# lijiaman/egoego_release

Measured on AMD Instinct MI355X. Metric: diffusion-steps/sec (B=256, T=120, 22-joint), higher is better.
Workload: dtype i8x3 + bf16x3 (attention layer, fc, FFN and linear_out: 2 x int8 slices per operand, int32 accumulate; embed: split-bf16, fp32 accumulate)

## Files before the change

egoego_release_amd/csrc/tail_fused.h:

```cpp
#pragma once
#include <type_traits>

#include "gemm.h"

#ifndef TAIL_ABLATE
#define TAIL_ABLATE 0
#endif
#ifndef TAIL_RING1
#define TAIL_RING1 4
#endif
#ifndef TAIL_RING_IO
#define TAIL_RING_IO 4
#endif
#ifndef TAIL8_RING
#define TAIL8_RING 4
#endif
#ifndef TAIL8_RING_FC
#define TAIL8_RING_FC 4
#endif

struct TailArgs {
    const __bf16* o;
    size_t o_plane;
    int HD16;
    const __bf16* wfc;
    size_t wfc_plane;
    EpiResLN<2, 4, 0> ln1;
    const __bf16* w1;
    size_t w1_plane;
    EpiTiled<true, 2> relu;
    const __bf16* w2;
    size_t w2_plane;
    EpiResLN<2, 4, 0> ln2;
    int fc8, H;
    const int8_t* o8;
    size_t o8_plane;
    const float* o_scale;
    const int8_t* wfc8;
    size_t wfc8_plane;
    const float* s_wfc;
    const int8_t* wfc8_3;
    int ffn8;
    const int8_t* w1_8;
    const int8_t* w2_8;
    size_t w8_plane;
    const float* s_w1;
    const float* s_w2;
    EpiReluQ8<4, 0> relu8;
    int stop;
    unsigned* outlier;
    int outlier_rows;
    EG_DBG(unsigned long long* trace;)
};

static constexpr int tail_smem_bytes(int TT, int NWV = 4) { return TT * 32 * 1024 + 3 * TT * NWV * 32 * TT * 4; }
static constexpr int TAIL_PAR_BYTES = 10 * 512 * 4;

using tail_rsrc = __amdgpu_buffer_rsrc_t;
EG_D tail_rsrc tail_make_rsrc(const void* p, size_t bytes) {
    return __builtin_amdgcn_make_buffer_rsrc((void*)p, 0, (int)(bytes < 0x7fffffffu ? bytes : 0x7fffffffu), 0x00020000);
}
EG_D i32x4 tail_load(tail_rsrc r, int voff, unsigned soff) {
    return __builtin_bit_cast(i32x4, __builtin_amdgcn_raw_buffer_load_b128(r, voff, soff, 0));
}

template <int FT, int TT, int RING, bool LAST, int DP, int NKS = 8, bool I8 = false, bool WLO0 = false>
struct TailChunk {
    using AccT = typename std::conditional<I8, I8Acc, f32x16>::type;
    static constexpr int PD = RING - 1, NW = FT * 2;
    static constexpr int NWL = WLO0 ? FT : NW;
    static_assert(!WLO0 || I8, "int8 slices only");
    static_assert(NKS == 8 || (LAST && DP == 0), "only the last chunk may be short");
    static_assert(RING == 2 || RING == 4 || RING == 8, "ring slots must divide the 8 k-steps of a chunk");
    static constexpr int n_ops(int s) { return ((s + PD < NKS || !LAST) ? NWL : 0) + (s == 0 ? DP : 0); }
    static constexpr int after_dma() {
        int n = 0;
        for (int s = 1; s < 8; ++s) n += n_ops(s);
        return n < 63 ? n : 63;
    }
    static constexpr int allowed(int ks) {
        int n = 0;
        if (ks < PD) {
            n += (PD - 1 - ks) * NWL;
            for (int s = 0; s < ks; ++s) n += n_ops(s);
        } else {
            n += ks - PD == 0 ? DP : 0;
            for (int s = ks - PD + 1; s < ks; ++s) n += n_ops(s);
        }
        return n < 63 ? n : 63;
    }
    template <int G>
    static EG_D void mma(i32x4 w, i32x4 a, f32x16& c) {
        if (TAIL_ABLATE & 8) return;
        c = __builtin_amdgcn_mfma_f32_32x32x16_bf16(__builtin_bit_cast(bf16x8, w), __builtin_bit_cast(bf16x8, a), c, 0, 0, 0);
    }
    template <int G>
    static EG_D void mma(i32x4 w, i32x4 a, I8Acc& c) {
        if (TAIL_ABLATE & 8) return;
        i32x16& d = G == 2 ? c.h : c.m;
        d = __builtin_amdgcn_mfma_i32_32x32x32_i8(w, a, d, 0, 0, 0);
    }

    template <int KS, class Dma>
    static EG_D void step(AccT (&acc)[FT][TT], i32x4 (&wq)[RING][NW], i32x4 (&ah)[2][TT], i32x4 (&al)[TT], tail_rsrc wr,
                          const unsigned (&wcur)[NW], const unsigned (&wnext)[NW], const char* act, int act_plane, int lane, Dma& dma) {
        constexpr int cur = KS & 1;
        asm volatile("" ::: "memory");
        wait_counts<allowed(KS), (KS == 0 ? 0 : TT)>();
        __builtin_amdgcn_sched_barrier(0);
        if (KS + PD < NKS || !LAST) {
            constexpr int kn = KS + PD;
#pragma unroll
            for (int q = 0; q < NW; ++q)
                if (!(TAIL_ABLATE & 1) && !(WLO0 && (q & 1))) wq[kn % RING][q] = tail_load(wr, lane * 16, kn < 8 ? wcur[q] + (kn << 10) : wnext[q] + ((kn & 7) << 10));
        }
        if (KS == 0 && DP) {
#pragma unroll
            for (int d = 0; d < DP; ++d)
                if (!(TAIL_ABLATE & 4)) dma(d);
        }
        if (KS < NKS - 1) {
#pragma unroll
            for (int j = 0; j < TT; ++j)
                if (!(TAIL_ABLATE & 2)) ah[cur ^ 1][j] = *(const i32x4*)(act + ((j * 8 + KS + 1) << 10) + lane * 16);
        }
        __builtin_amdgcn_sched_barrier(0);
        const i32x4(&w)[NW] = wq[KS % RING];
        if (!WLO0) {
#pragma unroll
            for (int i = 0; i < FT; ++i)
#pragma unroll
                for (int j = 0; j < TT; ++j) mma<0>(w[2 * i + 1], ah[cur][j], acc[i][j]);
        }
        asm volatile("" ::: "memory");
        wait_counts<63, (KS < NKS - 1 ? TT : 0)>();
        __builtin_amdgcn_sched_barrier(0);
#pragma unroll
        for (int i = 0; i < FT; ++i)
#pragma unroll
            for (int j = 0; j < TT; ++j) mma<1>(w[2 * i], al[j], acc[i][j]);
        __builtin_amdgcn_sched_barrier(0);
        if (KS < NKS - 1) {
#pragma unroll
            for (int j = 0; j < TT; ++j)
                if (!(TAIL_ABLATE & 2)) al[j] = *(const i32x4*)(act + act_plane + ((j * 8 + KS + 1) << 10) + lane * 16);
        }
        __builtin_amdgcn_sched_barrier(0);
#pragma unroll
        for (int i = 0; i < FT; ++i)
#pragma unroll
            for (int j = 0; j < TT; ++j) mma<2>(w[2 * i], ah[cur][j], acc[i][j]);
        __builtin_amdgcn_sched_barrier(0);
    }

    template <class Dma>
    static EG_D void run(AccT (&acc)[FT][TT], i32x4 (&wq)[RING][NW], tail_rsrc wr, const unsigned (&wcur)[NW],
                         const unsigned (&wnext)[NW], const char* act, int act_plane, int lane, Dma dma) {
        i32x4 ah[2][TT], al[TT];
#pragma unroll
        for (int j = 0; j < TT; ++j) {
            ah[0][j] = *(const i32x4*)(act + ((j * 8) << 10) + lane * 16);
            al[j] = *(const i32x4*)(act + act_plane + ((j * 8) << 10) + lane * 16);
        }
        step<0>(acc, wq, ah, al, wr, wcur, wnext, act, act_plane, lane, dma);
        if (NKS > 1) step<1>(acc, wq, ah, al, wr, wcur, wnext, act, act_plane, lane, dma);
        if (NKS > 2) step<2>(acc, wq, ah, al, wr, wcur, wnext, act, act_plane, lane, dma);
        if (NKS > 3) step<3>(acc, wq, ah, al, wr, wcur, wnext, act, act_plane, lane, dma);
        if (NKS > 4) step<4>(acc, wq, ah, al, wr, wcur, wnext, act, act_plane, lane, dma);
        if (NKS > 5) step<5>(acc, wq, ah, al, wr, wcur, wnext, act, act_plane, lane, dma);
        if (NKS > 6) step<6>(acc, wq, ah, al, wr, wcur, wnext, act, act_plane, lane, dma);
        if (NKS > 7) step<7>(acc, wq, ah, al, wr, wcur, wnext, act, act_plane, lane, dma);
        if (DP) {
            asm volatile("" ::: "memory");
            wait_counts<after_dma(), 15>();
        }
    }
};

template <int FT, int TT, int RING, bool REM2 = false, bool I8 = false, int NWAVES = 4, bool WLO0 = false>
struct DirectGemm {
    using AccT = typename std::conditional<I8, I8Acc, f32x16>::type;
    static constexpr int NW = 2 * FT, PD = RING - 1;
    static constexpr int CH_PLANE = TT * 8 * 1024, CH_BYTES = 2 * CH_PLANE;
    static constexpr int DMA_PIECES = 16 * TT / NWAVES;
    static constexpr int SMEM_BYTES = 2 * CH_BYTES;

    struct NoPost {
        EG_D void operator()(int) const {}
    };
    struct NoPre {
        EG_D void operator()() const {}
    };
    template <class Mark, class Post = NoPost, class Pre = NoPre>
    static EG_D void run(AccT (&acc)[FT][TT], const __bf16* in, size_t in_plane, int K16, const __bf16* w, size_t w_plane, char* act,
                         int tt0, int wave, int lane, Mark mark, int wtile0 = -1, Post post = Post{}, Pre pre = Pre{}) {
        const int wt0 = wtile0 >= 0 ? wtile0 : wave * FT;
        i32x4 wq[RING][NW];
        const tail_rsrc wr = tail_make_rsrc(w, w_plane * 4);
        const tail_rsrc ir = tail_make_rsrc((const char*)in + (((size_t)tt0 * (size_t)K16) << 10), 0x7fffffffu);
        const unsigned wpb = (unsigned)(w_plane * 2), ipb = (unsigned)(in_plane * 2);
        const int NQ = REM2 ? K16 / 8 + 1 : K16 / 8;
        auto w_offsets = [&](int kb, unsigned (&out)[NW]) {
#pragma unroll
            for (int i = 0; i < FT; ++i)
#pragma unroll
                for (int s = 0; s < 2; ++s) out[2 * i + s] = s * wpb + (unsigned)(((wt0 + i) * K16 + kb) << 10);
        };
        auto dma_piece = [&](int q, int piece) {
            const int x = wave * DMA_PIECES + piece;
            const int s = x / (8 * TT), j = (x >> 3) % TT;
            int kb = x & 7;
            if (REM2 && q == NQ - 1) kb &= 1;
            const unsigned src = s * ipb + (unsigned)((j * K16 + 8 * q + kb) << 10);
            char* dst = act + (q & 1) * CH_BYTES + s * CH_PLANE + ((j * 8 + kb) << 10);
            __builtin_amdgcn_raw_ptr_buffer_load_lds(ir, (__attribute__((address_space(3))) void*)dst, 16, lane * 16, src, 0, 0);
        };
        unsigned wcur[NW], wnext[NW];
#pragma unroll
        for (int pc = 0; pc < DMA_PIECES; ++pc) dma_piece(0, pc);
        w_offsets(0, wcur);
#pragma unroll
        for (int k = 0; k < PD; ++k)
#pragma unroll
            for (int q = 0; q < NW; ++q)
                if (!(WLO0 && (q & 1))) wq[k][q] = tail_load(wr, lane * 16, wcur[q] + (k << 10));
#pragma unroll
        for (int i = 0; i < FT; ++i)
#pragma unroll
            for (int j = 0; j < TT; ++j) acc_zero(acc[i][j]);
        pre();
        asm volatile("s_waitcnt vmcnt(0)" ::: "memory");
        __syncthreads();
        mark();
        for (int q = 0; q + 1 < NQ; ++q) {
            w_offsets(8 * q, wcur);
            w_offsets(8 * q + 8, wnext);
            TailChunk<FT, TT, RING, false, DMA_PIECES, 8, I8, WLO0>::run(acc, wq, wr, wcur, wnext, act + (q & 1) * CH_BYTES, CH_PLANE, lane,
                                                             [&](int piece) { dma_piece(q + 1, piece); });
            post(q);
            __builtin_amdgcn_s_barrier();
            asm volatile("" ::: "memory");
        }
        w_offsets(8 * (NQ - 1), wcur);
        TailChunk<FT, TT, RING, true, 0, (REM2 ? 2 : 8), I8, WLO0>::run(acc, wq, wr, wcur, wcur, act + ((NQ - 1) & 1) * CH_BYTES, CH_PLANE, lane, [](int) {});
        post(NQ - 1);
        __syncthreads();
    }

    static EG_D void prime(i32x4 (&wq)[RING][NW], const __bf16* w, size_t w_plane, int K16, int wt0, int lane) {
        const tail_rsrc wr = tail_make_rsrc(w, w_plane * 4);
        const unsigned wpb = (unsigned)(w_plane * 2);
#pragma unroll
        for (int k = 0; k < PD; ++k)
#pragma unroll
            for (int i = 0; i < FT; ++i)
#pragma unroll
                for (int sl = 0; sl < 2; ++sl) wq[k][2 * i + sl] = tail_load(wr, lane * 16, sl * wpb + (unsigned)(((wt0 + i) * K16 + k) << 10));
    }
    template <class Mark>
    static EG_D void run_resident(AccT (&acc)[FT][TT], i32x4 (&wq)[RING][NW], const __bf16* w, size_t w_plane, const char* act, int lane, Mark mark,
                                  int wt0) {
        static_assert(!REM2, "two whole chunks");
        constexpr int K16 = 16;
        const tail_rsrc wr = tail_make_rsrc(w, w_plane * 4);
        const unsigned wpb = (unsigned)(w_plane * 2);
        auto w_offsets = [&](int kb, unsigned (&out)[NW]) {
#pragma unroll
            for (int i = 0; i < FT; ++i)
#pragma unroll
                for (int sl = 0; sl < 2; ++sl) out[2 * i + sl] = sl * wpb + (unsigned)(((wt0 + i) * K16 + kb) << 10);
        };
        unsigned wcur[NW], wnext[NW];
#pragma unroll
        for (int i = 0; i < FT; ++i)
#pragma unroll
            for (int j = 0; j < TT; ++j) acc_zero(acc[i][j]);
        mark();
        w_offsets(0, wcur);
        w_offsets(8, wnext);
        TailChunk<FT, TT, RING, false, 0, 8, I8>::run(acc, wq, wr, wcur, wnext, act, CH_PLANE, lane, [](int) {});
        TailChunk<FT, TT, RING, true, 0, 8, I8>::run(acc, wq, wr, wnext, wnext, act + CH_BYTES, CH_PLANE, lane, [](int) {});
    }
};

static constexpr int TAIL_RES_BYTES = 272;
template <int TT, bool FFN8, bool FC8 = false, bool W2 = false, int NWV = 4, bool RES = false>
__global__ __launch_bounds__(64 * NWV, ((W2 || NWV == 8) ? 2 : 1)) void tail_kernel(TailArgs a) {
    static_assert(!RES || (FFN8 && FC8 && TT == 1), "LDS-resident FFN operands: the all-int8 32-token tail");
    static_assert(!W2 || (FFN8 && FC8 && TT == 1), "the two-workgroups-per-CU build exists for the all-int8 32-token tail");
    static_assert(NWV == 4 || (NWV == 8 && TT == 1 && !W2 && ((FFN8 && FC8) || (!FFN8 && !FC8 && !RES))),
                  "the eight-wave build exists for the 32-token tails: all int8, or (round 5) all split-bf16");
    constexpr int TOK = 32 * TT, FT = 16 / NWV;
    using G = DirectGemm<FT, TT, 4, false, false, NWV>;
    extern __shared__ __attribute__((aligned(16))) char smem[];
    char* const act = smem;
    char* const red = smem + G::SMEM_BYTES;
    const int wave = wave_id_uniform();
    const int lane = threadIdx.x & 63;
    const int tok0 = (int)blockIdx.x * TOK;
    const int tt0 = (int)blockIdx.x * TT;
    EG_DBG(unsigned long long* const tr = a.trace ? a.trace + 180224 + (size_t)blockIdx.x * 32 : nullptr;)
    auto mark = [&](int i) {
        EG_DBG(if (tr && threadIdx.x == 0) {
            tr[i] = wall_clock64();
            tr[16 + i] = __builtin_readcyclecounter();
        })
        (void)i;
    };
    mark(0);
    f32x16 acc[FT][TT];
    auto as_ln = [&](const EpiResLN<2, 4, 0>& e, int which = 0) {
        return EpiResLN<2, NWV, TOK>{e.bias, e.res, e.res_plane, e.gamma, e.beta, e.row_mask, e.out, e.out_plane, e.eps, e.q8, e.q8_plane, e.q8_scale, e.res8, e.res8_plane, e.res8_scale, nullptr, nullptr,
                                     a.outlier ? a.outlier + which : nullptr, nullptr, a.outlier_rows};
    };
    const float *p_swfc = a.s_wfc, *p_sw1 = a.s_w1, *p_sw2 = a.s_w2;
    const float* const par_src[10] = {a.s_wfc, a.ln1.bias, a.ln1.gamma, a.ln1.beta, a.s_w1, a.relu8.bias, a.s_w2, a.ln2.bias, a.ln2.gamma, a.ln2.beta};
    auto stage_params = [&] {
        float* par = (float*)(smem + tail_smem_bytes(TT, NWV));
        if (threadIdx.x < 128) {
#pragma unroll
            for (int v = 0; v < 10; ++v) *(float4*)(par + v * 512 + 4 * threadIdx.x) = *(const float4*)(par_src[v] + 4 * threadIdx.x);
        }
    };
    if constexpr (FFN8 && FC8) {
        float* par = (float*)(smem + tail_smem_bytes(TT, NWV));
        p_swfc = par;
        a.ln1.bias = par + 512; a.ln1.gamma = par + 1024; a.ln1.beta = par + 1536;
        p_sw1 = par + 2048; a.relu8.bias = par + 2560;
        p_sw2 = par + 3072; a.ln2.bias = par + 3584; a.ln2.gamma = par + 4096; a.ln2.beta = par + 4608;
    }

    if constexpr (FC8) {
        constexpr int FP = NWV == 8 ? 1 : ((W2 || TAIL_RING1 == 8) ? 2 : TT), FTP = FT / FP;
        using GF = DirectGemm<FTP, TT, (NWV == 8 ? TAIL8_RING_FC : (W2 ? 4 : TAIL_RING1)), false, true, NWV>;
        const int col = lane & 31;
#pragma unroll
        for (int i = 0; i < FT; ++i)
#pragma unroll
            for (int j = 0; j < TT; ++j)
#pragma unroll
                for (int r = 0; r < 16; ++r) acc[i][j][r] = 0.f;
#pragma unroll
        for (int fp = 0; fp < FP; ++fp) {
            I8Acc q[FTP][TT];
            GF::run(q, (const __bf16*)a.o8, a.o8_plane / 2, a.HD16 / 2, (const __bf16*)a.wfc8, a.wfc8_plane / 2, act, tt0, wave, lane, [&] { mark(7); },
                    wave * FT + fp * FTP, [&](int h) {
                        float so[TT];
#pragma unroll
                        for (int j = 0; j < TT; ++j) so[j] = a.o_scale[(size_t)(tok0 + j * 32 + col) * a.H + h] * 256.0f;
#pragma unroll
                        for (int i = 0; i < FTP; ++i)
#pragma unroll
                            for (int j = 0; j < TT; ++j) {
                                i8_fold(q[i][j], acc[fp * FTP + i][j], so[j]);
                                acc_zero(q[i][j]);
                            }
                    }, [&] { if (fp == 0) stage_params(); });
        }
        if (a.wfc8_3) {
#pragma unroll
            for (int fp = 0; fp < FP; ++fp) {
                I8Acc q[FTP][TT];
                using GF3 = DirectGemm<FTP, TT, (NWV == 8 ? TAIL8_RING_FC : (W2 ? 4 : TAIL_RING1)), false, true, NWV, true>;
                GF3::run(q, (const __bf16*)a.o8, a.o8_plane / 2, a.HD16 / 2, (const __bf16*)a.wfc8_3, a.wfc8_plane / 2, act, tt0, wave, lane, [&] {},
                        wave * FT + fp * FTP, [&](int h) {
                            float so[TT];
#pragma unroll
                            for (int j = 0; j < TT; ++j) so[j] = a.o_scale[(size_t)(tok0 + j * 32 + col) * a.H + h] * (1.0f / 256.0f);
#pragma unroll
                            for (int i = 0; i < FTP; ++i)
#pragma unroll
                                for (int j = 0; j < TT; ++j) {
                                    i8_fold(q[i][j], acc[fp * FTP + i][j], so[j]);
                                    acc_zero(q[i][j]);
                                }
                        });
            }
        }
#pragma unroll
        for (int i = 0; i < FT; ++i)
#pragma unroll
            for (int j = 0; j < TT; ++j) i8_fold_finish(acc[i][j], p_swfc + wave * FT * 32 + i * 32 + 4 * (lane >> 5));
    } else {
        G::run(acc, a.o, a.o_plane, a.HD16, a.wfc, a.wfc_plane, act, tt0, wave, lane, [&] { mark(7); });
    }
    mark(1);
    if constexpr (RES) {
        constexpr int FP8 = W2 ? 2 : 1, FTP8 = FT / FP8, RING8 = NWV == 8 ? TAIL8_RING : 4;
        using G8 = DirectGemm<FTP8, TT, RING8, false, true, NWV>;
        float* const ls1 = (float*)(smem + tail_smem_bytes(TT, NWV) + TAIL_PAR_BYTES);
        float* const ls2 = ls1 + 32;
        i32x4 wq[RING8][2 * FTP8];
        Rows8<FT> h1;
        auto ffn_resident = [&](I8Acc (&q)[FT][TT], const int8_t* w8, int mk) {
#pragma unroll
            for (int fp = 0; fp < FP8; ++fp) {
                if (fp) G8::prime(wq, (const __bf16*)w8, a.w8_plane / 2, 16, wave * FT + fp * FTP8, lane);
                G8::run_resident(*(I8Acc(*)[FTP8][TT]) & q[fp * FTP8], wq, (const __bf16*)w8, a.w8_plane / 2, act, lane, [&] { mark(mk); }, wave * FT + fp * FTP8);
            }
        };
        G8::prime(wq, (const __bf16*)a.w1_8, a.w8_plane / 2, 16, wave * FT, lane);
        {
            auto e = as_ln(a.ln1);
            if (a.stop != 1) { e.q8 = nullptr; e.q8_scale = nullptr; }
            e.lds_q8 = act; e.lds_scale = ls1;
            if (e.outlier) { e.outlier = nullptr; e.outlier_park = ls2 + 32; }
            e.template run<FT, TT, NoRows, Rows8<FT>>(acc, wave * FT * 32, tok0, lane, wave, 0, red, nullptr, &h1);
        }
        if (a.stop == 1) return;
        __syncthreads();
        mark(2);
        I8Acc q[FT][TT];
        ffn_resident(q, a.w1_8, 8);
        mark(3);
        G8::prime(wq, (const __bf16*)a.w2_8, a.w8_plane / 2, 16, wave * FT, lane);
        {
            const bool tap = a.stop == 2;
            const EpiReluQ8<NWV, TOK> e{a.relu8.bias, tap ? a.relu8.q8 : nullptr, a.relu8.q8_plane, tap ? a.relu8.q8_scale : nullptr, act, ls2, tap ? tok0 : 0};
            e.template run<false, I8Acc, FT, TT>(q, p_sw1, ls1, wave * FT * 32, 0, lane, wave, 0, red);
        }
        if (a.stop == 2) return;
        __syncthreads();
        mark(4);
        ffn_resident(q, a.w2_8, 9);
        mark(5);
        i8_dequant_tile<false>(q, acc, p_sw2, ls2, wave * FT * 32, 0, lane);
        {
            auto e = as_ln(a.ln2, 1);
            e.res8 = nullptr;
            e.template run<FT, TT, Rows8<FT>, NoRows>(acc, wave * FT * 32, tok0, lane, wave, 0, red, &h1, nullptr);
        }
        if (a.outlier && threadIdx.x == 0) atomicMax(a.outlier, __builtin_bit_cast(unsigned, ls2[32]));
        EG_DBG(if (tr) { asm volatile("s_waitcnt vmcnt(0)" ::: "memory"); })
        mark(6);
        return;
    }
    as_ln(a.ln1).template run<FT, TT>(acc, wave * FT * 32, tok0, lane, wave, 0, red);
    asm volatile("s_waitcnt vmcnt(0)" ::: "memory");
    __syncthreads();
    mark(2);
    if (a.stop == 1) return;

    if constexpr (FFN8) {
        constexpr int FP8 = NWV == 8 ? 1 : ((W2 || (TT == 1 && TAIL_RING1 == 8)) ? 2 : 1), FTP8 = FT / FP8;
        using G8 = DirectGemm<FTP8, TT, (TT == 2 ? 2 : (W2 ? 4 : (NWV == 8 ? TAIL8_RING : TAIL_RING1))), false, true, NWV>;
        const EpiReluQ8<NWV, TOK> e8{a.relu8.bias, a.relu8.q8, a.relu8.q8_plane, a.relu8.q8_scale};
        auto ffn_gemm = [&](I8Acc (&q)[FT][TT], const int8_t* in8, size_t in_plane_bytes, const int8_t* w8, int mk) {
#pragma unroll
            for (int fp = 0; fp < FP8; ++fp)
                G8::run(*(I8Acc(*)[FTP8][TT]) & q[fp * FTP8], (const __bf16*)in8, in_plane_bytes / 2, 16, (const __bf16*)w8, a.w8_plane / 2, act, tt0, wave,
                        lane, [&] { mark(mk); }, wave * FT + fp * FTP8);
        };
        {
            I8Acc q[FT][TT];
            ffn_gemm(q, a.ln1.q8, a.ln1.q8_plane, a.w1_8, 8);
            mark(3);
            e8.template run<false, I8Acc, FT, TT>(q, p_sw1, a.ln1.q8_scale, wave * FT * 32, tok0, lane, wave, 0, red);
        }
        asm volatile("s_waitcnt vmcnt(0)" ::: "memory");
        __syncthreads();
        mark(4);
        if (a.stop == 2) return;
        {
            I8Acc q[FT][TT];
            ffn_gemm(q, a.relu8.q8, a.relu8.q8_plane, a.w2_8, 9);
            mark(5);
            i8_dequant_tile<false>(q, acc, p_sw2, a.relu8.q8_scale, wave * FT * 32, tok0, lane);
        }
        as_ln(a.ln2, 1).template run<FT, TT>(acc, wave * FT * 32, tok0, lane, wave, 0, red);
        EG_DBG(if (tr) { asm volatile("s_waitcnt vmcnt(0)" ::: "memory"); })
        mark(6);
        return;
    }
    if constexpr (!FFN8) {
    G::run(acc, a.ln1.out, a.ln1.out_plane, 32, a.w1, a.w1_plane, act, tt0, wave, lane, [&] { mark(8); });
    mark(3);
    a.relu.template run<FT, TT>(acc, wave * FT * 32, tok0, lane, wave, 0, red);
    asm volatile("s_waitcnt vmcnt(0)" ::: "memory");
    __syncthreads();
    mark(4);
    if (a.stop == 2) return;

    G::run(acc, a.relu.out, a.relu.out_plane, 32, a.w2, a.w2_plane, act, tt0, wave, lane, [&] { mark(9); });
    mark(5);
    as_ln(a.ln2, 1).template run<FT, TT>(acc, wave * FT * 32, tok0, lane, wave, 0, red);
    EG_DBG(if (tr) { asm volatile("s_waitcnt vmcnt(0)" ::: "memory"); })
    mark(6);
    }
}

struct EmbedArgs {
    const __bf16* x;
    size_t x_plane;
    int K16;
    const __bf16* w;
    size_t w_plane;
    EpiEmbed<2, 4, 0> epi;
};
template <int TT, int NWV = 4>
__global__ __launch_bounds__(64 * NWV, (NWV == 8 ? 2 : 1)) void embed_kernel(EmbedArgs a) {
    constexpr int FT = 16 / NWV;
    using G = DirectGemm<FT, TT, TAIL_RING_IO, true, false, NWV>;
    extern __shared__ __attribute__((aligned(16))) char smem[];
    const int wave = wave_id_uniform(), lane = threadIdx.x & 63;
    f32x16 acc[FT][TT];
    G::run(acc, a.x, a.x_plane, a.K16, a.w, a.w_plane, smem, (int)blockIdx.x * TT, wave, lane, [] {});
    const EpiEmbed<2, NWV, 32 * TT> e{a.epi.bias, a.epi.pe, a.epi.tt_table, a.epi.t_idx, a.epi.out, a.epi.out_plane, a.epi.Lp, a.epi.T, a.epi.B,
                                      a.epi.q8, a.epi.q8_plane, a.epi.q8_scale, a.epi.state, a.epi.ts};
    e.template run<FT, TT>(acc, wave * FT * 32, (int)blockIdx.x * 32 * TT, lane, wave, 0, smem);
}

template <bool IDS = false>
struct OutArgsT {
    const __bf16* h;
    size_t h_plane;
    const __bf16* w;
    size_t w_plane;
    EpiOut<2, IDS> epi;
    const int8_t* h8;
    size_t h8_plane;
    const float* h_scale;
    const int8_t* w8;
    size_t w8_plane;
    const float* s_w;
};
template <int TT, int FS, bool I8 = false, bool IDS = false>
__global__ __launch_bounds__(256, 1) void out_kernel(OutArgsT<IDS> a) {
    constexpr int FT = 2 / FS;
    extern __shared__ __attribute__((aligned(16))) char smem[];
    const int wave = wave_id_uniform(), lane = threadIdx.x & 63;
    const int tb = (int)blockIdx.x / FS, fh = (int)blockIdx.x % FS;
    f32x16 acc[FT][TT];
    if constexpr (I8) {
        using G = DirectGemm<FT, TT, TAIL_RING_IO, false, true>;
        I8Acc q[FT][TT];
        G::run(q, (const __bf16*)a.h8, a.h8_plane / 2, 16, (const __bf16*)a.w8, a.w8_plane / 2, smem, tb * TT, wave, lane, [] {}, (fh * 4 + wave) * FT);
        i8_dequant_tile<false>(q, acc, a.s_w, a.h_scale, (fh * 4 + wave) * FT * 32, tb * 32 * TT, lane);
    } else {
        using G = DirectGemm<FT, TT, TAIL_RING_IO>;
        G::run(acc, a.h, a.h_plane, 32, a.w, a.w_plane, smem, tb * TT, wave, lane, [] {}, (fh * 4 + wave) * FT);
    }
    if constexpr (FS == 1) {
        a.epi.template run_block<FT, TT, 32 * TT, 256>(acc, wave * FT * 32, tb * 32 * TT, tb * 32 * TT, lane, smem);
    } else {
        a.epi.template run<FT, TT>(acc, (fh * 4 + wave) * FT * 32, tb * 32 * TT, lane, wave, 0, smem);
    }
}
```

Measured before the change: 736.5.

## Run int8 fc head-major across feature passes and stage o_scale in LDS

The int8 output-projection GEMM previously ran each feature pass (fp) as a separate full sweep over all heads, re-streaming the attention-output activation chunks through LDS once per pass. A new run_heads path iterates heads in the outer loop and all feature passes inside, so each activation chunk is DMA'd once and reused by every pass. A constexpr queue model statically checks that the counted vmcnt waits still match the new issue order. Per-token o_scale values are also transposed into shared memory during parameter staging, so the fold reads LDS instead of strided global memory. The cost is more complex wait accounting, extra LDS space, and a longer DMA wait that now spans all passes of a head.

```diff
diff --git a/egoego_release_amd/csrc/tail_fused.h b/egoego_release_amd/csrc/tail_fused.h
--- a/egoego_release_amd/csrc/tail_fused.h
+++ b/egoego_release_amd/csrc/tail_fused.h
@@ -54,7 +54,8 @@
 };
 
 static constexpr int tail_smem_bytes(int TT, int NWV = 4) { return TT * 32 * 1024 + 3 * TT * NWV * 32 * TT * 4; }
-static constexpr int TAIL_PAR_BYTES = 10 * 512 * 4;
+static constexpr int TAIL_PAR_FLOATS = 10 * 512, TAIL_OSC_FLOATS = 64 * 16;
+static constexpr int TAIL_PAR_BYTES = (TAIL_PAR_FLOATS + TAIL_OSC_FLOATS) * 4;
 
 using tail_rsrc = __amdgpu_buffer_rsrc_t;
 EG_D tail_rsrc tail_make_rsrc(const void* p, size_t bytes) {
@@ -64,7 +65,7 @@
     return __builtin_bit_cast(i32x4, __builtin_amdgcn_raw_buffer_load_b128(r, voff, soff, 0));
 }
 
-template <int FT, int TT, int RING, bool LAST, int DP, int NKS = 8, bool I8 = false, bool WLO0 = false>
+template <int FT, int TT, int RING, bool LAST, int DP, int NKS = 8, bool I8 = false, bool WLO0 = false, bool DMAWAIT = true>
 struct TailChunk {
     using AccT = typename std::conditional<I8, I8Acc, f32x16>::type;
     static constexpr int PD = RING - 1, NW = FT * 2;
@@ -72,7 +73,9 @@
     static_assert(!WLO0 || I8, "int8 slices only");
     static_assert(NKS == 8 || (LAST && DP == 0), "only the last chunk may be short");
     static_assert(RING == 2 || RING == 4 || RING == 8, "ring slots must divide the 8 k-steps of a chunk");
-    static constexpr int n_ops(int s) { return ((s + PD < NKS || !LAST) ? NWL : 0) + (s == 0 ? DP : 0); }
+    static constexpr bool loads_at(int s) { return s + PD < NKS || !LAST; }
+    static constexpr int dma_at(int s) { return s == 0 ? DP : 0; }
+    static constexpr int n_ops(int s) { return (loads_at(s) ? NWL : 0) + dma_at(s); }
     static constexpr int after_dma() {
         int n = 0;
         for (int s = 1; s < 8; ++s) n += n_ops(s);
@@ -108,15 +111,15 @@
         asm volatile("" ::: "memory");
         wait_counts<allowed(KS), (KS == 0 ? 0 : TT)>();
         __builtin_amdgcn_sched_barrier(0);
-        if (KS + PD < NKS || !LAST) {
+        if (loads_at(KS)) {
             constexpr int kn = KS + PD;
 #pragma unroll
             for (int q = 0; q < NW; ++q)
                 if (!(TAIL_ABLATE & 1) && !(WLO0 && (q & 1))) wq[kn % RING][q] = tail_load(wr, lane * 16, kn < 8 ? wcur[q] + (kn << 10) : wnext[q] + ((kn & 7) << 10));
         }
-        if (KS == 0 && DP) {
-#pragma unroll
-            for (int d = 0; d < DP; ++d)
+        if (dma_at(KS)) {
+#pragma unroll
+            for (int d = 0; d < dma_at(KS); ++d)
                 if (!(TAIL_ABLATE & 4)) dma(d);
         }
         if (KS < NKS - 1) {
@@ -170,10 +173,52 @@
         if (NKS > 5) step<5>(acc, wq, ah, al, wr, wcur, wnext, act, act_plane, lane, dma);
         if (NKS > 6) step<6>(acc, wq, ah, al, wr, wcur, wnext, act, act_plane, lane, dma);
         if (NKS > 7) step<7>(acc, wq, ah, al, wr, wcur, wnext, act, act_plane, lane, dma);
-        if (DP) {
+        if (DP && DMAWAIT) {
             asm volatile("" ::: "memory");
             wait_counts<after_dma(), 15>();
         }
+    }
+};
+
+template <int FT, int TT, int RING, int DP, bool I8, bool WLO0, int FP, int NH>
+struct FcQueueModel {
+    using First = TailChunk<FT, TT, RING, false, DP, 8, I8, WLO0, false>;
+    using Mid = TailChunk<FT, TT, RING, false, 0, 8, I8, WLO0>;
+    using Last = TailChunk<FT, TT, RING, true, 0, 8, I8, WLO0>;
+    static constexpr int PD = RING - 1, NWL = First::NWL, NSEG = NH * FP;
+    static constexpr int clamp63(int n) { return n < 63 ? n : 63; }
+    static constexpr int check(int dma_wait) {
+        int issued = 0, waits = 0;
+        int w_end[NSEG + 1][8] = {};
+        int d_end[NH + 1] = {};
+        issued += DP;
+        d_end[0] = issued;
+        for (int k = 0; k < PD; ++k) {
+            issued += NWL;
+            w_end[0][k] = issued;
+        }
+        for (int seg = 0; seg < NSEG; ++seg) {
+            const int h = seg / FP, fp = seg % FP;
+            const bool last = seg == NSEG - 1, first = fp == 0 && h + 1 < NH;
+            for (int ks = 0; ks < 8; ++ks) {
+                const int n = last ? Last::allowed(ks) : (first ? First::allowed(ks) : Mid::allowed(ks));
+                ++waits;
+                if (n != clamp63(issued - w_end[seg][ks])) return waits;
+                if (last ? Last::loads_at(ks) : (first ? First::loads_at(ks) : Mid::loads_at(ks))) {
+                    issued += NWL;
+                    w_end[ks + PD < 8 ? seg : seg + 1][(ks + PD) & 7] = issued;
+                }
+                if (first && First::dma_at(ks)) {
+                    issued += First::dma_at(ks);
+                    d_end[h + 1] = issued;
+                }
+            }
+            if (fp == FP - 1 && h + 1 < NH) {
+                ++waits;
+                if (dma_wait != clamp63(issued - d_end[h + 1])) return waits;
+            }
+        }
+        return 0;
     }
 };
 
@@ -244,6 +289,78 @@
         w_offsets(8 * (NQ - 1), wcur);
         TailChunk<FT, TT, RING, true, 0, (REM2 ? 2 : 8), I8, WLO0>::run(acc, wq, wr, wcur, wcur, act + ((NQ - 1) & 1) * CH_BYTES, CH_PLANE, lane, [](int) {});
         post(NQ - 1);
+        __syncthreads();
+    }
+
+    template <int FP>
+    static constexpr int heads_dma_wait() {
+        constexpr int n = (7 + 8 * (FP - 1)) * (WLO0 ? FT : NW);
+        return n < 63 ? n : 63;
+    }
+    template <int FP, int fp, bool LASTH, class Post, class Dma>
+    static EG_D void head_passes(AccT (&q)[FT][TT], i32x4 (&wq)[RING][NW], tail_rsrc wr, unsigned wpb, int K16, int wtile0, int h, const char* buf, int lane,
+                                 Post& post, Dma dma) {
+        auto w_offsets = [&](int p, int kb, unsigned (&out)[NW]) {
+#pragma unroll
+            for (int i = 0; i < FT; ++i)
+#pragma unroll
+                for (int s = 0; s < 2; ++s) out[2 * i + s] = s * wpb + (unsigned)(((wtile0 + p * FT + i) * K16 + kb) << 10);
+        };
+        unsigned wcur[NW], wnext[NW];
+        w_offsets(fp, 8 * h, wcur);
+        if (fp + 1 < FP) w_offsets(fp + 1, 8 * h, wnext);
+        else w_offsets(0, 8 * h + 8, wnext);
+        if constexpr (LASTH && fp == FP - 1) TailChunk<FT, TT, RING, true, 0, 8, I8, WLO0>::run(q, wq, wr, wcur, wcur, buf, CH_PLANE, lane, [](int) {});
+        else if constexpr (!LASTH && fp == 0) TailChunk<FT, TT, RING, false, DMA_PIECES, 8, I8, WLO0, false>::run(q, wq, wr, wcur, wnext, buf, CH_PLANE, lane, dma);
+        else TailChunk<FT, TT, RING, false, 0, 8, I8, WLO0>::run(q, wq, wr, wcur, wnext, buf, CH_PLANE, lane, [](int) {});
+        post(h, std::integral_constant<int, fp>{});
+        if constexpr (fp + 1 < FP) head_passes<FP, fp + 1, LASTH>(q, wq, wr, wpb, K16, wtile0, h, buf, lane, post, dma);
+    }
+    template <int FP, class Mark, class Post, class Pre>
+    static EG_D void run_heads(AccT (&q)[FT][TT], const __bf16* in, size_t in_plane, int K16, const __bf16* w, size_t w_plane, char* act, int tt0, int wave,
+                               int lane, Mark mark, int wtile0, Post post, Pre pre) {
+        static_assert(I8 && !REM2 && FP > 1, "the int8 fc in several feature passes");
+        static_assert(FcQueueModel<FT, TT, RING, DMA_PIECES, I8, WLO0, FP, 1>::check(heads_dma_wait<FP>()) == 0 &&
+                          FcQueueModel<FT, TT, RING, DMA_PIECES, I8, WLO0, FP, 2>::check(heads_dma_wait<FP>()) == 0 &&
+                          FcQueueModel<FT, TT, RING, DMA_PIECES, I8, WLO0, FP, 4>::check(heads_dma_wait<FP>()) == 0,
+                      "a counted wait of the head-major fc does not match the order its loads are issued in");
+        i32x4 wq[RING][NW];
+        const tail_rsrc wr = tail_make_rsrc(w, w_plane * 4);
+        const tail_rsrc ir = tail_make_rsrc((const char*)in + (((size_t)tt0 * (size_t)K16) << 10), 0x7fffffffu);
+        const unsigned wpb = (unsigned)(w_plane * 2), ipb = (unsigned)(in_plane * 2);
+        const int NQ = K16 / 8;
+        auto dma_piece = [&](int c, int piece) {
+            const int x = wave * DMA_PIECES + piece;
+            const int s = x / (8 * TT), j = (x >> 3) % TT, kb = x & 7;
+            const unsigned src = s * ipb + (unsigned)((j * K16 + 8 * c + kb) << 10);
+            char* dst = act + (c & 1) * CH_BYTES + s * CH_PLANE + ((j * 8 + kb) << 10);
+            __builtin_amdgcn_raw_ptr_buffer_load_lds(ir, (__attribute__((address_space(3))) void*)dst, 16, lane * 16, src, 0, 0);
+        };
+#pragma unroll
+        for (int pc = 0; pc < DMA_PIECES; ++pc) dma_piece(0, pc);
+#pragma unroll
+        for (int k = 0; k < PD; ++k)
+#pragma unroll
+            for (int i = 0; i < FT; ++i)
+#pragma unroll
+                for (int s = 0; s < 2; ++s)
+                    if (!(WLO0 && s)) wq[k][2 * i + s] = tail_load(wr, lane * 16, s * wpb + (unsigned)(((wtile0 + i) * K16 + k) << 10));
+#pragma unroll
+        for (int i = 0; i < FT; ++i)
+#pragma unroll
+            for (int j = 0; j < TT; ++j) acc_zero(q[i][j]);
+        pre();
+        asm volatile("s_waitcnt vmcnt(0)" ::: "memory");
+        __syncthreads();
+        mark();
+        for (int h = 0; h + 1 < NQ; ++h) {
+            head_passes<FP, 0, false>(q, wq, wr, wpb, K16, wtile0, h, act + (h & 1) * CH_BYTES, lane, post, [&](int piece) { dma_piece(h + 1, piece); });
+            asm volatile("" ::: "memory");
+            wait_counts<heads_dma_wait<FP>(), 15>();
+            __builtin_amdgcn_s_barrier();
+            asm volatile("" ::: "memory");
+        }
+        head_passes<FP, 0, true>(q, wq, wr, wpb, K16, wtile0, NQ - 1, act + ((NQ - 1) & 1) * CH_BYTES, lane, post, [](int) {});
         __syncthreads();
     }
 
@@ -320,6 +437,10 @@
         if (threadIdx.x < 128) {
 #pragma unroll
             for (int v = 0; v < 10; ++v) *(float4*)(par + v * 512 + 4 * threadIdx.x) = *(const float4*)(par_src[v] + 4 * threadIdx.x);
+            if constexpr (FC8) {
+                const float* const src = a.o_scale + (size_t)tok0 * a.H;
+                for (int x = threadIdx.x; x < TOK * a.H; x += 128) par[TAIL_PAR_FLOATS + (x % a.H) * TOK + x / a.H] = src[x];
+            }
         }
     };
     if constexpr (FFN8 && FC8) {
@@ -332,55 +453,48 @@
 
     if constexpr (FC8) {
         constexpr int FP = NWV == 8 ? 1 : ((W2 || TAIL_RING1 == 8) ? 2 : TT), FTP = FT / FP;
-        using GF = DirectGemm<FTP, TT, (NWV == 8 ? TAIL8_RING_FC : (W2 ? 4 : TAIL_RING1)), false, true, NWV>;
-        const int col = lane & 31;
+        constexpr int RING_FC = NWV == 8 ? TAIL8_RING_FC : (W2 ? 4 : TAIL_RING1);
+        EG_DBG(unsigned long long fold_ticks = 0;)
+        const float* const osc = (const float*)(smem + tail_smem_bytes(TT, NWV)) + TAIL_PAR_FLOATS + (lane & 31);
 #pragma unroll
         for (int i = 0; i < FT; ++i)
 #pragma unroll
             for (int j = 0; j < TT; ++j)
 #pragma unroll
                 for (int r = 0; r < 16; ++r) acc[i][j][r] = 0.f;
-#pragma unroll
-        for (int fp = 0; fp < FP; ++fp) {
+        auto fc_slices = [&](auto wlo0, const int8_t* w8, float unit, auto mark7, auto pre) {
+            using GF = DirectGemm<FTP, TT, RING_FC, false, true, NWV, decltype(wlo0)::value>;
             I8Acc q[FTP][TT];
-            GF::run(q, (const __bf16*)a.o8, a.o8_plane / 2, a.HD16 / 2, (const __bf16*)a.wfc8, a.wfc8_plane / 2, act, tt0, wave, lane, [&] { mark(7); },
-                    wave * FT + fp * FTP, [&](int h) {
-                        float so[TT];
-#pragma unroll
-                        for (int j = 0; j < TT; ++j) so[j] = a.o_scale[(size_t)(tok0 + j * 32 + col) * a.H + h] * 256.0f;
-#pragma unroll
-                        for (int i = 0; i < FTP; ++i)
-#pragma unroll
-                            for (int j = 0; j < TT; ++j) {
-                                i8_fold(q[i][j], acc[fp * FTP + i][j], so[j]);
-                                acc_zero(q[i][j]);
-                            }
-                    }, [&] { if (fp == 0) stage_params(); });
-        }
-        if (a.wfc8_3) {
-#pragma unroll
-            for (int fp = 0; fp < FP; ++fp) {
-                I8Acc q[FTP][TT];
-                using GF3 = DirectGemm<FTP, TT, (NWV == 8 ? TAIL8_RING_FC : (W2 ? 4 : TAIL_RING1)), false, true, NWV, true>;
-                GF3::run(q, (const __bf16*)a.o8, a.o8_plane / 2, a.HD16 / 2, (const __bf16*)a.wfc8_3, a.wfc8_plane / 2, act, tt0, wave, lane, [&] {},
-                        wave * FT + fp * FTP, [&](int h) {
-                            float so[TT];
-#pragma unroll
-                            for (int j = 0; j < TT; ++j) so[j] = a.o_scale[(size_t)(tok0 + j * 32 + col) * a.H + h] * (1.0f / 256.0f);
-#pragma unroll
-                            for (int i = 0; i < FTP; ++i)
-#pragma unroll
-                                for (int j = 0; j < TT; ++j) {
-                                    i8_fold(q[i][j], acc[fp * FTP + i][j], so[j]);
-                                    acc_zero(q[i][j]);
-                                }
-                        });
+            auto fold = [&](int h, auto fpc) {
+                constexpr int fp = decltype(fpc)::value;
+                EG_DBG(const unsigned long long c0 = __builtin_readcyclecounter();)
+                float so[TT];
+#pragma unroll
+                for (int j = 0; j < TT; ++j) so[j] = osc[h * TOK + j * 32] * unit;
+#pragma unroll
+                for (int i = 0; i < FTP; ++i)
+#pragma unroll
+                    for (int j = 0; j < TT; ++j) {
+                        i8_fold(q[i][j], acc[fp * FTP + i][j], so[j]);
+                        acc_zero(q[i][j]);
+                    }
+                EG_DBG(fold_ticks += __builtin_readcyclecounter() - c0;)
+            };
+            if constexpr (FP > 1) {
+                GF::template run_heads<FP>(q, (const __bf16*)a.o8, a.o8_plane / 2, a.HD16 / 2, (const __bf16*)w8, a.wfc8_plane / 2, act, tt0, wave, lane, mark7,
+                                           wave * FT, fold, pre);
+            } else {
+                GF::run(q, (const __bf16*)a.o8, a.o8_plane / 2, a.HD16 / 2, (const __bf16*)w8, a.wfc8_plane / 2, act, tt0, wave, lane, mark7, wave * FT,
+                        [&](int h) { fold(h, std::integral_constant<int, 0>{}); }, pre);
             }
-        }
+        };
+        fc_slices(std::false_type{}, a.wfc8, 256.0f, [&] { mark(7); }, [&] { stage_params(); });
+        if (a.wfc8_3) fc_slices(std::true_type{}, a.wfc8_3, 1.0f / 256.0f, [] {}, [] {});
 #pragma unroll
         for (int i = 0; i < FT; ++i)
 #pragma unroll
             for (int j = 0; j < TT; ++j) i8_fold_finish(acc[i][j], p_swfc + wave * FT * 32 + i * 32 + 4 * (lane >> 5));
+        EG_DBG(if (tr && threadIdx.x == 0) tr[10] = fold_ticks;)
     } else {
         G::run(acc, a.o, a.o_plane, a.HD16, a.wfc, a.wfc_plane, act, tt0, wave, lane, [&] { mark(7); });
     }
```

Result: faster. 748.4 (median of 6 runs) (+1.6%).
